# GATB/leon

Hardware: AMD Instinct MI355X
Metric: compressed input MB/s (DNA encode path) (higher is better)
Workload: dtype u64

## Files before the change

### leon_amd/csrc/host_rc.h

```cpp
#pragma once
#include <stdint.h>
#if defined(__x86_64__)
#include <emmintrin.h>
#define LEON_HOST_CHAIN_X86 1
#endif
#include <pthread.h>
#include <sched.h>
#if defined(__linux__)
#include <sys/mman.h>
#endif
#include <chrono>
#include <cstdio>
#include <condition_variable>
#include <cstdlib>
#include <cstring>
#include <new>
#include <algorithm>
#include <deque>
#include <memory>
#include <mutex>
#include <thread>
#include <type_traits>
#include <vector>

namespace leon {

class ReciprocalStream {
public:
    static constexpr uint64_t kChunk = 1ull << 18;
    static constexpr uint32_t kBufs = 12, kThreads = 3;
    ReciprocalStream() { for (auto& b : buf_) b.resize(kChunk); }
    ~ReciprocalStream() { stop(); }
    void restart() {
        stop();
        consumed_ = 0; quit_ = false;
        for (auto& h : holds_) h = 0;
        for (uint32_t j = 0; j < kThreads; j++) th_[j] = std::thread([this, j] { run(j); });
        running_ = true;
    }
    void stop() {
        if (!running_) return;
        { std::lock_guard<std::mutex> g(mu_); quit_ = true; }
        cv_.notify_all();
        for (auto& t : th_) t.join();
        running_ = false;
    }
    const uint64_t* take(uint64_t c) {
        std::unique_lock<std::mutex> g(mu_);
        if (c > consumed_) { consumed_ = c; cv_.notify_all(); }
        cv_.wait(g, [&] { return holds_[c % kBufs] == c + 1; });
        return buf_[c % kBufs].data();
    }
    static inline uint64_t reciprocal(uint64_t d) {
        if (d <= 256) return 0;
#ifdef LEON_HOST_CHAIN_X86
        uint64_t q, r;
        asm("divq %[d]" : "=a"(q), "=d"(r) : "a"(~0ull), "d"(255ull), [d] "r"(d) : "cc");
        return q;
#else
        return (uint64_t)(((((unsigned __int128)255) << 64) | ~0ull) / d);
#endif
    }
private:
    void run(uint32_t j) {
        for (uint64_t c = j;; c += kThreads) {
            {
                std::unique_lock<std::mutex> g(mu_);
                cv_.wait(g, [&] { return quit_ || c < consumed_ + kBufs; });
                if (quit_) return;
            }
            uint64_t* out = buf_[c % kBufs].data();
            const uint64_t t0 = c * kChunk;
            for (uint64_t i = 0; i < kChunk; i++) out[i] = reciprocal(5 + t0 + i);
            { std::lock_guard<std::mutex> g(mu_); holds_[c % kBufs] = c + 1; }
            cv_.notify_all();
        }
    }
    std::vector<uint64_t> buf_[kBufs];
    uint64_t holds_[kBufs] = {};
    std::mutex mu_;
    std::condition_variable cv_;
    uint64_t consumed_ = 0;
    bool quit_ = false, running_ = false;
    std::thread th_[kThreads];
};


struct ChainCpus {
    bool use = false;
    cpu_set_t set;
    void pick() {
        const char* e = getenv("LEON_CHAIN_PIN");
        if (!e || e[0] != '1') return;
        const int cpu = sched_getcpu();
        if (cpu < 0) return;
        char path[128];
        snprintf(path, sizeof path, "/sys/devices/system/cpu/cpu%d/cache/index3/shared_cpu_list", cpu);
        FILE* f = fopen(path, "r");
        if (!f) return;
        char line[1024];
        const bool ok = fgets(line, sizeof line, f) != nullptr;
        fclose(f);
        if (!ok) return;
        cpu_set_t l3, allowed;
        CPU_ZERO(&l3);
        for (char* p = line; *p && *p != '\n';) {
            char* q = nullptr;
            const long a = strtol(p, &q, 10);
            if (q == p) break;
            long b = a;
            if (*q == '-') { p = q + 1; b = strtol(p, &q, 10); }
            for (long c = a; c <= b && c < CPU_SETSIZE; c++) if (c >= 0) CPU_SET((int)c, &l3);
            p = *q == ',' ? q + 1 : q;
            if (*q != ',') break;
        }
        if (sched_getaffinity(0, sizeof allowed, &allowed) != 0) return;
        CPU_AND(&set, &l3, &allowed);
        use = CPU_COUNT(&set) >= 7;
    }
    void apply() const { if (use) (void)pthread_setaffinity_np(pthread_self(), sizeof set, &set); }
};

struct ChainRec16 { uint64_t c; uint32_t lo, fr; };
struct ChainRec24 { uint64_t c, lo, fr; };
struct ChainRecCarry { uint64_t c, qmm; uint32_t lo, fr; };

constexpr int kChainPrefetchBytes = 2048;

class ChainRing {
public:
    ChainRing() = default;
    ChainRing(const ChainRing&) = delete;
    ChainRing& operator=(const ChainRing&) = delete;
    ~ChainRing() { free(p_); }
    bool allocated() const { return p_ != nullptr; }
    size_t stride() const { return stride_; }
    void allocate(uint32_t n, size_t stride, bool huge) {
        constexpr size_t kHuge = (size_t)2 << 20;
        stride_ = (stride + 63) & ~(size_t)63;
        const size_t bytes = ((size_t)n * stride_ + kHuge - 1) & ~(kHuge - 1);
        void* q = nullptr;
        if (posix_memalign(&q, kHuge, bytes) != 0) throw std::bad_alloc();
        p_ = static_cast<char*>(q);
#if defined(__linux__) && defined(MADV_HUGEPAGE)
        if (huge) (void)madvise(p_, bytes, MADV_HUGEPAGE);
#else
        (void)huge;
#endif
    }
    void* at(uint32_t b) const { return p_ + (size_t)b * stride_; }
private:
    char* p_ = nullptr;
    size_t stride_ = 0;
};

class ChainFeed {
public:
    static constexpr uint32_t kMaxBufs = 1024;
    static constexpr uint64_t kPlainBelow = 512;
    struct View {
        const void* recs = nullptr; uint64_t n_syms = 0;
        bool wide = false, carry = false;
        const uint64_t* kmers = nullptr; uint32_t n_kmers = 0;
        uint64_t t0 = 0;
        uint64_t c_end[4] = {};
    };
    explicit ChainFeed(uint32_t k) : k_(k), W_(k >= 32 ? 2u : 1u), seg_kmers_(std::max<uint32_t>(1, (1u << 15) / k)) {
        carry_ = kCarryByDefault;
        if (const char* e = getenv("LEON_CHAIN_FORM")) { if (!strcmp(e, "carry")) carry_ = true; else if (!strcmp(e, "quotient")) carry_ = false; }
#ifdef LEON_HOST_CHAIN_X86
        if (carry_ && !__builtin_cpu_supports("bmi2")) carry_ = false;
#else
        carry_ = false;
#endif
        if (const char* e = getenv("LEON_CHAIN_HUGEPAGES")) huge_ = e[0] == '1';
        uint32_t n = carry_ ? 4 : 3, spares = 3;
        if (const char* e = getenv("LEON_CHAIN_HELPERS")) { const int v = atoi(e); if (v >= 1 && v <= 32) n = (uint32_t)v; }
        if (const char* e = getenv("LEON_CHAIN_SPARES")) { const int v = atoi(e); if (v >= 0 && v <= 32) spares = (uint32_t)v; }
        n_threads_ = n; n_spares_ = spares;
        if (const char* e = getenv("LEON_CHAIN_RING")) { const int v = atoi(e); if (v >= 4 && v <= (int)kMaxBufs) n_bufs_ = (uint32_t)v; }
    }
    ~ChainFeed() { stop(); }
    static constexpr bool kCarryByDefault = true;
    bool carry() const { return carry_; }
    ChainCpus cpus_;
    void start() {
        if (running_) return;
        quit_ = false;
        if (!ring_.allocated()) ring_.allocate(n_bufs_, (size_t)seg_kmers_ * k_ * (carry_ ? sizeof(ChainRecCarry) : sizeof(ChainRec16)), huge_);
        for (uint32_t j = 0; j < n_threads_ + n_spares_; j++) th_.emplace_back([this, j] { run(j >= n_threads_); });
        running_ = true;
    }
    void stop() {
        if (!running_) return;
        { std::lock_guard<std::mutex> g(mu_); quit_ = true; }
        cv_work_.notify_all(); cv_spare_.notify_all(); cv_ready_.notify_all();
        for (auto& t : th_) t.join();
        th_.clear();
        running_ = false;
    }
    void reset_stream() {
        std::lock_guard<std::mutex> g(mu_);
        segs_.clear(); base_ = 0; next_claim_ = 0; next_take_ = 0; released_ = 0; prefix_upto_ = 0; t_pushed_ = 0;
        for (auto& c : prefix_c_) c = 1;
        for (auto& r : ready_) r = 0;
    }
    uint32_t push(const uint64_t* kmers, size_t count) {
        uint32_t n = 0;
        {
            std::lock_guard<std::mutex> g(mu_);
            while (count) {
                const bool plain = t_pushed_ < kPlainBelow;
                const size_t take = plain ? std::min<size_t>(count, (kPlainBelow - t_pushed_ + k_ - 1) / k_) : std::min<size_t>(count, seg_kmers_);
                Seg sg; sg.kmers = kmers; sg.n_kmers = (uint32_t)take; sg.plain = plain; sg.t0 = t_pushed_;
                sg.wide = t_pushed_ + take * k_ + 8 >= (1ull << 32);
                segs_.push_back(sg);
                kmers += take * W_; count -= take; t_pushed_ += take * k_; n++;
            }
        }
        cv_work_.notify_all(); cv_spare_.notify_all();
        return n;
    }
    void take(View& v) {
        std::unique_lock<std::mutex> g(mu_);
        const uint64_t s = next_take_++;
        if (n_spares_ && (int64_t)(next_claim_ - next_take_) < (int64_t)low_water()) cv_spare_.notify_all();
        cv_ready_.wait(g, [&] { return ready_[s % n_bufs_] == s + 1; });
        const Seg& sg = segs_[s - base_];
        v.recs = sg.plain ? nullptr : slot(sg.wide, s);
        v.wide = sg.wide; v.carry = carry_ && !sg.wide;
        v.n_syms = (uint64_t)sg.n_kmers * k_; v.kmers = sg.kmers; v.n_kmers = sg.n_kmers; v.t0 = sg.t0;
        for (int i = 0; i < 4; i++) v.c_end[i] = sg.c_end[i];
    }
    void release() {
        { std::lock_guard<std::mutex> g(mu_); released_++; while (base_ < released_ && !segs_.empty()) { segs_.pop_front(); base_++; } }
        cv_work_.notify_all();
    }
private:
    struct Seg { const uint64_t* kmers; uint32_t n_kmers; bool plain, wide; uint64_t t0; uint64_t c0[4], c_end[4]; };
    static inline void count_codes(uint64_t x, uint64_t* n) {
        const uint64_t lo = x & 0x5555555555555555ull, hi = (x >> 1) & 0x5555555555555555ull;
        n[1] += (uint64_t)__builtin_popcountll(lo & ~hi); n[2] += (uint64_t)__builtin_popcountll(hi & ~lo); n[3] += (uint64_t)__builtin_popcountll(lo & hi);
    }
    uint64_t low_water() const { return n_bufs_ / 4; }
    void run(bool spare) {
        cpus_.apply();
        for (;;) {
            uint64_t s; Seg sg;
            {
                std::unique_lock<std::mutex> g(mu_);
                auto work = [&] { return next_claim_ < base_ + segs_.size() && next_claim_ < released_ + n_bufs_; };
                if (spare) cv_spare_.wait(g, [&] { return quit_ || (work() && (int64_t)(next_claim_ - next_take_) < (int64_t)low_water()); });
                else cv_work_.wait(g, [&] { return quit_ || work(); });
                if (quit_) return;
                s = next_claim_++;
                sg = segs_[s - base_];
            }
            uint64_t h[4] = {0, 0, 0, 0};
            for (uint32_t a = 0; a < sg.n_kmers; a++) for (uint32_t w = 0; w < W_; w++) count_codes(sg.kmers[(size_t)a * W_ + w], h);
            h[0] = (uint64_t)sg.n_kmers * k_ - h[1] - h[2] - h[3];
            uint64_t c[4];
            {
                std::unique_lock<std::mutex> g(mu_);
                cv_prefix_.wait(g, [&] { return quit_ || prefix_upto_ == s; });
                if (quit_) return;
                for (int i = 0; i < 4; i++) { c[i] = prefix_c_[i]; prefix_c_[i] += h[i]; }
                prefix_upto_ = s + 1;
                Seg& d = segs_[s - base_];
                for (int i = 0; i < 4; i++) { d.c0[i] = c[i]; d.c_end[i] = prefix_c_[i]; }
            }
            cv_prefix_.notify_all();
            if (!sg.plain) {
                if (sg.wide) {
                    { std::lock_guard<std::mutex> g(mu_); if (!wide_ring().allocated()) wide_ring_.allocate(n_bufs_, (size_t)seg_kmers_ * k_ * sizeof(ChainRec24), huge_); }
                    fill(static_cast<ChainRec24*>(slot(true, s)), sg, c);
                } else if (carry_) fill(static_cast<ChainRecCarry*>(slot(false, s)), sg, c);
                else fill(static_cast<ChainRec16*>(slot(false, s)), sg, c);
            }
            { std::lock_guard<std::mutex> g(mu_); ready_[s % n_bufs_] = s + 1; }
            cv_ready_.notify_all();
        }
    }
    static inline uint64_t scaled(uint64_t fr, uint64_t d) {
#ifdef LEON_HOST_CHAIN_X86
        uint64_t q, r;
        asm("divq %[d]" : "=a"(q), "=d"(r) : "a"(0ull), "d"(fr), [d] "r"(d) : "cc");
        return q;
#else
        return (uint64_t)((((unsigned __int128)fr) << 64) / d);
#endif
    }
    static inline uint64_t qmm_of(uint64_t fr) {
        constexpr uint64_t kNum = (1ull << 56) - 1;
        uint64_t m = (uint64_t)(int64_t)(0x1p56 / (double)(int64_t)fr);
        int64_t r = (int64_t)(kNum - m * fr);
        if (r < 0) { m--; r += (int64_t)fr; }
        if (r >= (int64_t)fr) { m++; r -= (int64_t)fr; }
        if (__builtin_expect((uint64_t)r >= fr, 0)) m = kNum / fr;
        return m;
    }
    template <typename Rec> void fill(Rec* out, const Seg& sg, uint64_t* c) const {
        uint64_t d = 5 + sg.t0 + 1;
        uint64_t cum[5] = {0, c[0], c[0] + c[1], c[0] + c[1] + c[2], c[0] + c[1] + c[2] + c[3]};
        for (uint32_t a = 0; a < sg.n_kmers; a++) {
            const uint64_t* w = sg.kmers + (size_t)a * W_;
            unsigned __int128 x = W_ == 2 ? (((unsigned __int128)w[1] << 64) | w[0]) << (128 - 2 * k_) : (unsigned __int128)w[0] << (128 - 2 * k_);
            for (uint32_t i = 0; i < k_; i++, d++, out++, x <<= 2) {
                const uint32_t sy = (uint32_t)(x >> 126);
                const uint64_t lo = cum[sy], fr = cum[sy + 1] - lo;
                out->c = scaled(fr, d);
                if constexpr (std::is_same<Rec, ChainRecCarry>::value) out->qmm = qmm_of(fr);
                out->lo = (decltype(out->lo))lo; out->fr = (decltype(out->fr))fr;
                cum[1] += sy < 1; cum[2] += sy < 2; cum[3] += sy < 3; cum[4]++;
            }
        }
        c[0] = cum[1]; c[1] = cum[2] - cum[1]; c[2] = cum[3] - cum[2]; c[3] = cum[4] - cum[3];
    }
    const uint32_t k_, W_, seg_kmers_;
    uint32_t n_threads_ = 5;
    ChainRing& wide_ring() { return ring_.stride() >= (size_t)seg_kmers_ * k_ * sizeof(ChainRec24) ? ring_ : wide_ring_; }
    void* slot(bool wide, uint64_t s) { return (wide ? wide_ring() : ring_).at((uint32_t)(s % n_bufs_)); }
    ChainRing ring_, wide_ring_;
    bool carry_ = false, huge_ = false;
    uint64_t ready_[kMaxBufs] = {};
    uint32_t n_bufs_ = 512, n_spares_ = 0;
    std::condition_variable cv_spare_;
    std::deque<Seg> segs_;
    uint64_t base_ = 0, next_claim_ = 0, next_take_ = 0, released_ = 0, prefix_upto_ = 0, t_pushed_ = 0;
    uint64_t prefix_c_[4] = {1, 1, 1, 1};
    std::mutex mu_;
    std::condition_variable cv_work_, cv_prefix_, cv_ready_;
    bool quit_ = false, running_ = false;
    std::vector<std::thread> th_;
};

class ByteBuf {
public:
    ~ByteBuf() { free(p_); }
    uint8_t* data() { return p_; }
    const uint8_t* data() const { return p_; }
    size_t size() const { return cap_; }
    void clear() {}
    void resize(size_t n) {
        if (n <= cap_) return;
        uint8_t* q = (uint8_t*)realloc(p_, n);
        if (!q) throw std::bad_alloc();
        p_ = q; cap_ = n;
    }
    uint8_t& operator[](size_t i) { return p_[i]; }
private:
    uint8_t* p_ = nullptr;
    size_t cap_ = 0;
};

class AnchorDictCoder {
public:
    AnchorDictCoder() { clear(); }
    void clear() {
        low_ = 0; range_ = ~0ull; n_ = 0; buf_.clear(); w_ = 0;
        for (int i = 0; i <= 5; i++) cum_[i] = i;
    }
    void encode_kmers(const uint64_t* w, size_t count, uint32_t k) {
        const uint32_t W = k >= 32 ? 2u : 1u;
        for (; count; count--, w += W) encode_kmer_plain(w, k);
    }
    inline void encode_kmer(const uint64_t* w, uint32_t k) { encode_kmers(w, 1, k); }
    inline void encode_kmer_plain(const uint64_t* w, uint32_t k) {
        if (buf_.size() < w_ + 8 * (size_t)k + 16) buf_.resize(buf_.size() * 2 + 8 * (size_t)k + 4096);
        for (uint32_t i = 0; i < k; i++) {
            const uint32_t bit = 2 * (k - 1 - i);
            encode((uint32_t)(w[bit >> 6] >> (bit & 63)) & 3u);
        }
    }
    void encode_segment(const ChainFeed::View& v, uint32_t k) {
#ifdef LEON_HOST_CHAIN_X86
        if (v.recs) {
            if (v.wide) encode_records(static_cast<const ChainRec24*>(v.recs), v.n_syms, v.t0);
            else if (v.carry) encode_records_carry(static_cast<const ChainRecCarry*>(v.recs), v.n_syms, v.t0);
            else encode_records(static_cast<const ChainRec16*>(v.recs), v.n_syms, v.t0);
            for (int i = 0; i < 4; i++) cum_[i + 1] = cum_[i] + v.c_end[i];
            cum_[5] = cum_[4] + 1;
            return;
        }
#endif
        encode_kmers(v.kmers, v.n_kmers, k);
    }
    void flush() {
        if (buf_.size() < w_ + 24) buf_.resize(w_ + 24);
        settle();
        for (int i = 0; i < 8; i++) { buf_[w_++] = (uint8_t)(low_ >> 56); low_ <<= 8; }
    }
    const uint8_t* data() const { return buf_.data(); }
    size_t size() const { return w_; }
    uint64_t symbols() const { return n_; }
private:
#ifdef LEON_HOST_CHAIN_X86
    template <typename Rec, int kAhead = kChainPrefetchBytes> void encode_records(const Rec* r, uint64_t n, uint64_t t0) {
        if (buf_.size() < w_ + 8 * n + 64) buf_.resize(buf_.size() * 2 + 8 * n + 4096);
        settle();
        uint8_t* p = buf_.data() + w_;
        uint8_t* p_end = buf_.data() + buf_.size() - 32;
        uint64_t L = low_, R = range_, tot1 = 5 + t0;
        uint64_t q = R / tot1;
        const Rec* const e = r + n;
        for (; r < e; r++) {
            tot1++;
            __builtin_prefetch(reinterpret_cast<const char*>(r) + kAhead);
            const uint64_t lo = r->lo, lf = lo + r->fr;
            const uint64_t Lu = L + q * lo;
            uint64_t Tu = L + q * lf;
            asm("" : "+r"(Tu));
            const uint64_t Ru = Tu - Lu, x = Lu ^ Tu;
            const uint64_t q8 = q << 8;
            const unsigned __int128 P = (unsigned __int128)q * r->c;
            const uint64_t Phi = (uint64_t)(P >> 64), Plo = (uint64_t)P, Phi8 = (Phi << 8) | (Plo >> 56), Plo8 = Plo << 8;
            if (__builtin_expect((x >> 48) == 0 || Ru < kBottom, 0)) {
                L = Lu; R = Ru;
                while ((L ^ (L + R)) < kTop || (R < kBottom && ((R = (0 - L) & (kBottom - 1)), true))) {
                    if (p >= p_end) { const size_t used = (size_t)(p - buf_.data()); buf_.resize(buf_.size() * 2 + 4096); p = buf_.data() + used; p_end = buf_.data() + buf_.size() - 32; }
                    *p++ = (uint8_t)(L >> 56);
                    R <<= 8;
                    L <<= 8;
                }
                q = R / tot1;
                continue;
            }
            uint64_t qn = Phi, Ln = Lu;
            R = Ru;
            *p = (uint8_t)(Lu >> 56);
            asm("cmpq %[top], %[x]\n\tcmovbq %[A], %[qn]\n\tcmovbq %[R1], %[R]\n\tcmovbq %[L1], %[Ln]\n\tadcq $0, %[p]"
                : [qn] "+r"(qn), [R] "+r"(R), [Ln] "+r"(Ln), [p] "+r"(p)
                : [x] "r"(x), [top] "r"(kTop), [A] "r"(Phi8), [R1] "r"(Ru << 8), [L1] "r"(Lu << 8)
                : "cc");
            if (__builtin_expect((Plo + q < q) | (Plo8 + q8 < q8), 0)) qn = R / tot1;
            q = qn; L = Ln;
        }
        w_ = (size_t)(p - buf_.data());
        low_ = L; range_ = R; n_ += n;
    }
    struct PlainStep { uint64_t q, L, R; uint8_t* p; };
    __attribute__((noinline)) PlainStep step_plain(const ChainRecCarry* r, uint64_t tot_next, uint64_t q, uint64_t L, uint8_t* p) {
        uint64_t Lo = L + q * r->lo, R = q * r->fr;
        uint8_t* p_end = buf_.data() + buf_.size() - 32;
        while ((Lo ^ (Lo + R)) < kTop || (R < kBottom && ((R = (0 - Lo) & (kBottom - 1)), true))) {
            if (p >= p_end) { const size_t used = (size_t)(p - buf_.data()); buf_.resize(buf_.size() * 2 + 4096); p = buf_.data() + used; p_end = buf_.data() + buf_.size() - 32; }
            *p++ = (uint8_t)(Lo >> 56);
            R <<= 8;
            Lo <<= 8;
        }
        return PlainStep{R / tot_next, Lo, R, p};
    }
#define LEON_CARRY_STEP(OFF, LIN, LOUT, LOUT32, EXIT)                                                                  \
                "movq  %%rdx, %%r14\n\t"                                  \
                "mulxq " OFF "(%[r]), %%rbx, %%rbx\n\t"                                                         \
                "movl  " OFF "+16(%[r]), " LOUT32 "\n\t"                                                         \
                "movl  " OFF "+20(%[r]), %%r13d\n\t"                                                             \
                "shlxq %[eight], " LOUT ", %%r12\n\t"                                                       \
                "shlxq %[eight], %%r13, %%r13\n\t"                                                          \
                "imulq %%rdx, %%r12\n\t"                                                              \
                "imulq %%rdx, %%r13\n\t"                                                         \
                "imulq %%rdx, " LOUT "\n\t"                                                                  \
                "cmpq  %%rdx, " OFF "+8(%[r])\n\t"                          \
                "sbbq  %%rax, %%rax\n\t"                                                                               \
                "orq   %%rax, %%r13\n\t"                                                              \
                "shlxq %[eight], %%rdx, %%rax\n\t"                                                               \
                "mulq  " OFF "(%[r])\n\t"                                            \
                "cmpq  %[dbt], %%rax\n\t"                                                                              \
                "ja    " EXIT "\n\t"                                                              \
                "shlxq %[eight], " LIN ", %%rax\n\t"                                                         \
                "addq  %%rax, %%r12\n\t"                                                    \
                "addq  " LIN ", " LOUT "\n\t"                                                                    \
                "cmpq  %[top], %%r13\n\t"                                                                              \
                "jb    " EXIT "\n\t"                                                               \
                "rorxq $56, " LOUT ", %%rax\n\t"                                                                       \
                "movb  %%al, (%[p])\n\t"                                     \
                "stc\n\t"                                                                                              \
                "adcq  %%r12, %%r13\n\t"                            \
                "cmovcq %%rbx, %%rdx\n\t"                                        \
                "cmovncq %%r12, " LOUT "\n\t"                                          \
                "sbbq  $-1, %[p]\n\t"
    template <int kAhead = kChainPrefetchBytes> void encode_records_carry(const ChainRecCarry* r, uint64_t n, uint64_t t0) {
        if (!n) return;
        if (buf_.size() < w_ + 8 * n + 64) buf_.resize(buf_.size() * 2 + 8 * n + 4096);
        settle();
        uint8_t* p = buf_.data() + w_;
        uint64_t L = low_;
        const ChainRecCarry* const r0 = r;
        uint64_t q = range_ / (5 + t0);
        const ChainRecCarry* const e = r + n - 1;
        const ChainRecCarry* const e2 = e - 1;
        const uint64_t doubt_above = ~(uint64_t)((((unsigned __int128)1) << 72) / (5 + t0));
        while (r < e) {
            if (r < e2) {
                asm volatile(
                    ".p2align 5\n"
                    "1:\n\t"
                    LEON_CARRY_STEP("0", "%[L]", "%%rcx", "%%ecx", "2f")
                    LEON_CARRY_STEP("24", "%%rcx", "%[L]", "%k[L]", "3f")
                    "prefetcht0 %c[ahead](%[r])\n\t"
                    "addq  $48, %[r]\n\t"
                    "cmpq  %[e], %[r]\n\t"
                    "jb    1b\n\t"
                    "jmp   4f\n"
                    "3:\n\t"
                    "movq  %%rcx, %[L]\n\t"
                    "addq  $24, %[r]\n"
                    "2:\n\t"
                    "movq  %%r14, %%rdx\n"
                    "4:\n"
                    : [r] "+r"(r), [q] "+d"(q), [L] "+r"(L), [p] "+r"(p)
                    : [e] "m"(e2), [top] "r"(kTop), [dbt] "r"(doubt_above), [eight] "r"((uint64_t)8), [ahead] "i"(kAhead)
                    : "rax", "rbx", "rcx", "r12", "r13", "r14", "cc", "memory");
            }
            if (r >= e) break;
            const PlainStep s = step_plain(r, 5 + t0 + (uint64_t)(r - r0) + 1, q, L, p);
            q = s.q; L = s.L; p = s.p;
            r++;
        }
        const PlainStep s = step_plain(r, 5 + t0 + n, q, L, p);
        w_ = (size_t)(s.p - buf_.data());
        low_ = s.L; range_ = s.R; n_ += n;
    }
#undef LEON_CARRY_STEP
#endif
    inline void settle() {
        uint8_t* p = buf_.data() + w_;
        while ((low_ ^ (low_ + range_)) < kTop || (range_ < kBottom && ((range_ = (0 - low_) & (kBottom - 1)), true))) {
            *p++ = (uint8_t)(low_ >> 56);
            range_ <<= 8;
            low_ <<= 8;
        }
        w_ = (size_t)(p - buf_.data());
    }
    inline void encode(uint32_t c) {
        settle();
        const uint64_t lo = cum_[c], fr = cum_[c + 1] - cum_[c], tot = cum_[5];
        const uint64_t q = range_ / tot;
        low_ += lo * q;
        range_ = q * fr;
        for (uint32_t i = 1; i <= 5; i++) cum_[i] += (uint64_t)(i > c);
        n_++;
    }
    static constexpr uint64_t kTop = 1ull << 56, kBottom = 1ull << 48;
    uint64_t low_, range_, n_, cum_[6];
    ByteBuf buf_;
    size_t w_;
};

inline bool decode_anchor_dict(const uint8_t* p, uint64_t n, uint64_t n_anchors, uint32_t k, uint64_t* out) {
    constexpr uint64_t kTop = 1ull << 56, kBottom = 1ull << 48;
    const uint32_t W = k >= 32 ? 2u : 1u;
    uint64_t low = 0, range = ~0ull, code = 0, i = 0, t = 0, cum[6] = {0, 1, 2, 3, 4, 5};
    for (int b = 0; b < 8; b++) code = (code << 8) | (i < n ? p[i] : 0), i++;
    ReciprocalStream recips;
    const bool use_inv = n_anchors * (uint64_t)k > (1u << 16);
    if (use_inv) recips.restart();
    const uint64_t* inv = nullptr;
    uint64_t inv_chunk = ~0ull;
    auto recip_of_symbol = [&](uint64_t tt) -> uint64_t {
        const uint64_t c = tt / ReciprocalStream::kChunk;
        if (c != inv_chunk) { inv = recips.take(c); inv_chunk = c; }
        return inv[tt % ReciprocalStream::kChunk];
    };
    auto next_byte = [&]() -> uint64_t { const uint64_t v = i < n ? p[i] : 0; i++; return v; };
    uint64_t r = 0;
    bool r_valid = false;
    for (uint64_t a = 0; a < n_anchors; a++) {
        unsigned __int128 km = 0;
        for (uint32_t j = 0; j < k; j++, t++) {
            const uint64_t tot = 5 + t;
            if (!r_valid) r = range / tot;
            if (r == 0) return false;
            const uint64_t d = code - low;
            const uint64_t p1 = r * cum[1], p2 = r * cum[2], p3 = r * cum[3], p4 = r * cum[4];
            const bool g1 = d >= p1, g2 = d >= p2, g3 = d >= p3, g4 = d >= p4;
            if (g4) return false;
            const uint64_t R0 = p1, R1 = p2 - p1, R2 = p3 - p2, R3 = p4 - p3;
            const uint32_t c = (uint32_t)g1 + (uint32_t)g2 + (uint32_t)g3;
            uint64_t lo, R, h = 0;
            const bool fast = use_inv && t >= 256;
            if (fast) {
                const uint64_t m1 = recip_of_symbol(t + 1);
                uint64_t h0 = (uint64_t)(((unsigned __int128)R0 * m1) >> 64), h1 = (uint64_t)(((unsigned __int128)R1 * m1) >> 64);
                uint64_t h2 = (uint64_t)(((unsigned __int128)R2 * m1) >> 64), h3 = (uint64_t)(((unsigned __int128)R3 * m1) >> 64);
                const uint64_t lo_a = g1 ? p1 : 0, R_a = g1 ? R1 : R0, h_a = g1 ? h1 : h0;
                const uint64_t lo_b = g3 ? p3 : p2, R_b = g3 ? R3 : R2, h_b = g3 ? h3 : h2;
                lo = g2 ? lo_b : lo_a; R = g2 ? R_b : R_a; h = g2 ? h_b : h_a;
            } else {
                lo = g3 ? p3 : g2 ? p2 : g1 ? p1 : 0;
                R = g3 ? R3 : g2 ? R2 : g1 ? R1 : R0;
            }
            low += lo;
            range = R;
            const uint64_t x = low ^ (low + range);
            if (__builtin_expect(!fast || (x >> 48) == 0 || range < kBottom, 0)) {
                while ((low ^ (low + range)) < kTop || (range < kBottom && ((range = (0 - low) & (kBottom - 1)), true))) {
                    code = (code << 8) | next_byte();
                    range <<= 8;
                    low <<= 8;
                    if (i > n + 16) return false;
                }
                r_valid = false;
            } else {
                const uint64_t byte = i < n ? p[i] : 0;
                const uint64_t tot1 = tot + 1;
                uint64_t rn = h >> 8;
#ifdef LEON_HOST_CHAIN_X86
                asm("cmpq %[top], %[x]\n\tcmovbq %[h], %[rn]\n\tcmovbq %[R8], %[rg]\n\tcmovbq %[L8], %[lw]\n\tcmovbq %[C8], %[cd]\n\tadcq $0, %[i]"
                    : [rn] "+r"(rn), [rg] "+r"(range), [lw] "+r"(low), [cd] "+r"(code), [i] "+r"(i)
                    : [x] "r"(x), [top] "r"(kTop), [h] "r"(h), [R8] "r"(range << 8), [L8] "r"(low << 8), [C8] "r"((code << 8) | byte)
                    : "cc");
#else
                const bool one = x < kTop;
                rn = one ? h : rn; range = one ? range << 8 : range; low = one ? low << 8 : low; code = one ? (code << 8) | byte : code; i += one;
#endif
                if (__builtin_expect(range - rn * tot1 >= tot1, 0)) rn++;
                r = rn; r_valid = true;
            }
            cum[1] += (uint64_t)(c < 1); cum[2] += (uint64_t)(c < 2); cum[3] += (uint64_t)(c < 3); cum[4] += 1; cum[5] += 1;
            km = (km << 2) | c;
        }
        out[a * W] = (uint64_t)km;
        if (W == 2) out[a * W + 1] = (uint64_t)(km >> 64);
    }
    return true;
}

class AnchorDictWorker {
public:
    explicit AnchorDictWorker(uint32_t k) : k_(k), feed_(k) {}
    ~AnchorDictWorker() { stop(); feed_.stop(); }
    void push(std::vector<uint64_t>&& kmers) {
        const uint32_t W = k_ >= 32 ? 2u : 1u;
        {
            std::lock_guard<std::mutex> g(mu_);
            if (!running_) { running_ = true; quit_ = false; feed_.cpus_.pick(); feed_.start(); th_ = std::thread([this] { feed_.cpus_.apply(); run(); }); }
            q_.emplace_back(std::move(kmers), 0u);
            q_.back().second = feed_.push(q_.back().first.data(), q_.back().first.size() / W);
            pending_++;
        }
        cv_.notify_all();
    }
    void drain() {
        std::unique_lock<std::mutex> g(mu_);
        cv_done_.wait(g, [this] { return pending_ == 0; });
    }
    void stop() {
        {
            std::lock_guard<std::mutex> g(mu_);
            if (!running_) return;
            quit_ = true;
        }
        cv_.notify_all();
        th_.join();
        running_ = false;
    }
    void reset() { drain(); coder_.clear(); feed_.reset_stream(); busy_ms_ = 0; starved_ms_ = 0; }
    double busy_ms() const { return busy_ms_; }
    double starved_ms() const { return starved_ms_; }
    AnchorDictCoder& coder() { return coder_; }
private:
    void run() {
        for (;;) {
            std::pair<std::vector<uint64_t>, uint32_t> batch;
            {
                std::unique_lock<std::mutex> g(mu_);
                cv_.wait(g, [this] { return quit_ || !q_.empty(); });
                if (q_.empty()) return;
                batch = std::move(q_.front());
                q_.pop_front();
            }
            const auto t0 = std::chrono::steady_clock::now();
            for (uint32_t sgm = 0; sgm < batch.second; sgm++) {
                ChainFeed::View v;
                const auto tw = std::chrono::steady_clock::now();
                feed_.take(v);
                starved_ms_ += std::chrono::duration<double, std::milli>(std::chrono::steady_clock::now() - tw).count();
                coder_.encode_segment(v, k_);
                feed_.release();
            }
            busy_ms_ += std::chrono::duration<double, std::milli>(std::chrono::steady_clock::now() - t0).count();
            {
                std::lock_guard<std::mutex> g(mu_);
                pending_--;
            }
            cv_done_.notify_all();
        }
    }
    uint32_t k_;
    ChainFeed feed_;
    AnchorDictCoder coder_;
    std::mutex mu_;
    std::condition_variable cv_, cv_done_;
    std::deque<std::pair<std::vector<uint64_t>, uint32_t>> q_;
    uint64_t pending_ = 0;
    double busy_ms_ = 0, starved_ms_ = 0;
    bool running_ = false, quit_ = false;
    std::thread th_;
};

}
```

Before: 20680.

## Add shifted-quotient chain record form with new asm encode loop as default

Adds a third precomputed record form in which the quotient-multiplier is stored pre-shifted by 8 bits with low bits set, plus a hand-written inline-asm range-coder step that carries the quotient left-shifted. This removes shift instructions from the serial encode dependency chain and folds the renormalisation into fewer ops. The new form becomes the default. The risk is subtle arithmetic correctness in the new asm, with slow-path fallbacks when the quotient estimate is in doubt.

```diff
diff --git a/leon_amd/csrc/host_rc.h b/leon_amd/csrc/host_rc.h
--- a/leon_amd/csrc/host_rc.h
+++ b/leon_amd/csrc/host_rc.h
@@ -124,6 +124,8 @@
 struct ChainRec16 { uint64_t c; uint32_t lo, fr; };
 struct ChainRec24 { uint64_t c, lo, fr; };
 struct ChainRecCarry { uint64_t c, qmm; uint32_t lo, fr; };
+struct ChainRecShifted { uint64_t c, qmm8; uint32_t lo, fr; };
+enum class ChainForm { quotient, carry, shifted };
 
 constexpr int kChainPrefetchBytes = 2048;
 
@@ -160,34 +162,36 @@
     static constexpr uint64_t kPlainBelow = 512;
     struct View {
         const void* recs = nullptr; uint64_t n_syms = 0;
-        bool wide = false, carry = false;
+        bool wide = false; ChainForm form = ChainForm::quotient;
         const uint64_t* kmers = nullptr; uint32_t n_kmers = 0;
         uint64_t t0 = 0;
         uint64_t c_end[4] = {};
     };
     explicit ChainFeed(uint32_t k) : k_(k), W_(k >= 32 ? 2u : 1u), seg_kmers_(std::max<uint32_t>(1, (1u << 15) / k)) {
-        carry_ = kCarryByDefault;
-        if (const char* e = getenv("LEON_CHAIN_FORM")) { if (!strcmp(e, "carry")) carry_ = true; else if (!strcmp(e, "quotient")) carry_ = false; }
+        form_ = kDefaultForm;
+        if (const char* e = getenv("LEON_CHAIN_FORM")) {
+            if (!strcmp(e, "shifted")) form_ = ChainForm::shifted; else if (!strcmp(e, "carry")) form_ = ChainForm::carry; else if (!strcmp(e, "quotient")) form_ = ChainForm::quotient;
+        }
 #ifdef LEON_HOST_CHAIN_X86
-        if (carry_ && !__builtin_cpu_supports("bmi2")) carry_ = false;
+        if (form_ != ChainForm::quotient && !__builtin_cpu_supports("bmi2")) form_ = ChainForm::quotient;
 #else
-        carry_ = false;
+        form_ = ChainForm::quotient;
 #endif
         if (const char* e = getenv("LEON_CHAIN_HUGEPAGES")) huge_ = e[0] == '1';
-        uint32_t n = carry_ ? 4 : 3, spares = 3;
+        uint32_t n = form_ != ChainForm::quotient ? 4 : 3, spares = 3;
         if (const char* e = getenv("LEON_CHAIN_HELPERS")) { const int v = atoi(e); if (v >= 1 && v <= 32) n = (uint32_t)v; }
         if (const char* e = getenv("LEON_CHAIN_SPARES")) { const int v = atoi(e); if (v >= 0 && v <= 32) spares = (uint32_t)v; }
         n_threads_ = n; n_spares_ = spares;
         if (const char* e = getenv("LEON_CHAIN_RING")) { const int v = atoi(e); if (v >= 4 && v <= (int)kMaxBufs) n_bufs_ = (uint32_t)v; }
     }
     ~ChainFeed() { stop(); }
-    static constexpr bool kCarryByDefault = true;
-    bool carry() const { return carry_; }
+    static constexpr ChainForm kDefaultForm = ChainForm::shifted;
+    ChainForm form() const { return form_; }
     ChainCpus cpus_;
     void start() {
         if (running_) return;
         quit_ = false;
-        if (!ring_.allocated()) ring_.allocate(n_bufs_, (size_t)seg_kmers_ * k_ * (carry_ ? sizeof(ChainRecCarry) : sizeof(ChainRec16)), huge_);
+        if (!ring_.allocated()) ring_.allocate(n_bufs_, (size_t)seg_kmers_ * k_ * (form_ != ChainForm::quotient ? sizeof(ChainRecCarry) : sizeof(ChainRec16)), huge_);
         for (uint32_t j = 0; j < n_threads_ + n_spares_; j++) th_.emplace_back([this, j] { run(j >= n_threads_); });
         running_ = true;
     }
@@ -228,7 +232,7 @@
         cv_ready_.wait(g, [&] { return ready_[s % n_bufs_] == s + 1; });
         const Seg& sg = segs_[s - base_];
         v.recs = sg.plain ? nullptr : slot(sg.wide, s);
-        v.wide = sg.wide; v.carry = carry_ && !sg.wide;
+        v.wide = sg.wide; v.form = form_;
         v.n_syms = (uint64_t)sg.n_kmers * k_; v.kmers = sg.kmers; v.n_kmers = sg.n_kmers; v.t0 = sg.t0;
         for (int i = 0; i < 4; i++) v.c_end[i] = sg.c_end[i];
     }
@@ -274,7 +278,8 @@
                 if (sg.wide) {
                     { std::lock_guard<std::mutex> g(mu_); if (!wide_ring().allocated()) wide_ring_.allocate(n_bufs_, (size_t)seg_kmers_ * k_ * sizeof(ChainRec24), huge_); }
                     fill(static_cast<ChainRec24*>(slot(true, s)), sg, c);
-                } else if (carry_) fill(static_cast<ChainRecCarry*>(slot(false, s)), sg, c);
+                } else if (form_ == ChainForm::shifted) fill(static_cast<ChainRecShifted*>(slot(false, s)), sg, c);
+                else if (form_ == ChainForm::carry) fill(static_cast<ChainRecCarry*>(slot(false, s)), sg, c);
                 else fill(static_cast<ChainRec16*>(slot(false, s)), sg, c);
             }
             { std::lock_guard<std::mutex> g(mu_); ready_[s % n_bufs_] = s + 1; }
@@ -310,6 +315,7 @@
                 const uint64_t lo = cum[sy], fr = cum[sy + 1] - lo;
                 out->c = scaled(fr, d);
                 if constexpr (std::is_same<Rec, ChainRecCarry>::value) out->qmm = qmm_of(fr);
+                if constexpr (std::is_same<Rec, ChainRecShifted>::value) out->qmm8 = (qmm_of(fr) << 8) | 255;
                 out->lo = (decltype(out->lo))lo; out->fr = (decltype(out->fr))fr;
                 cum[1] += sy < 1; cum[2] += sy < 2; cum[3] += sy < 3; cum[4]++;
             }
@@ -321,7 +327,8 @@
     ChainRing& wide_ring() { return ring_.stride() >= (size_t)seg_kmers_ * k_ * sizeof(ChainRec24) ? ring_ : wide_ring_; }
     void* slot(bool wide, uint64_t s) { return (wide ? wide_ring() : ring_).at((uint32_t)(s % n_bufs_)); }
     ChainRing ring_, wide_ring_;
-    bool carry_ = false, huge_ = false;
+    ChainForm form_ = ChainForm::quotient;
+    bool huge_ = false;
     uint64_t ready_[kMaxBufs] = {};
     uint32_t n_bufs_ = 512, n_spares_ = 0;
     std::condition_variable cv_spare_;
@@ -376,7 +383,8 @@
 #ifdef LEON_HOST_CHAIN_X86
         if (v.recs) {
             if (v.wide) encode_records(static_cast<const ChainRec24*>(v.recs), v.n_syms, v.t0);
-            else if (v.carry) encode_records_carry(static_cast<const ChainRecCarry*>(v.recs), v.n_syms, v.t0);
+            else if (v.form == ChainForm::shifted) encode_records_shifted(static_cast<const ChainRecShifted*>(v.recs), v.n_syms, v.t0);
+            else if (v.form == ChainForm::carry) encode_records_carry(static_cast<const ChainRecCarry*>(v.recs), v.n_syms, v.t0);
             else encode_records(static_cast<const ChainRec16*>(v.recs), v.n_syms, v.t0);
             for (int i = 0; i < 4; i++) cum_[i + 1] = cum_[i] + v.c_end[i];
             cum_[5] = cum_[4] + 1;
@@ -439,7 +447,7 @@
         low_ = L; range_ = R; n_ += n;
     }
     struct PlainStep { uint64_t q, L, R; uint8_t* p; };
-    __attribute__((noinline)) PlainStep step_plain(const ChainRecCarry* r, uint64_t tot_next, uint64_t q, uint64_t L, uint8_t* p) {
+    template <typename Rec> __attribute__((noinline)) PlainStep step_plain(const Rec* r, uint64_t tot_next, uint64_t q, uint64_t L, uint8_t* p) {
         uint64_t Lo = L + q * r->lo, R = q * r->fr;
         uint8_t* p_end = buf_.data() + buf_.size() - 32;
         while ((Lo ^ (Lo + R)) < kTop || (R < kBottom && ((R = (0 - Lo) & (kBottom - 1)), true))) {
@@ -522,6 +530,74 @@
         low_ = s.L; range_ = s.R; n_ += n;
     }
 #undef LEON_CARRY_STEP
+#define LEON_SHIFTED_STEP(OFF, LIN, LOUT, LOUT32, EXIT)                                                                \
+                "mulxq " OFF "(%[r]), %%rax, %%rbx\n\t"                              \
+                "cmpq  %[dbt], %%rax\n\t"                                                                              \
+                "ja    " EXIT "\n\t"                                                              \
+                "movl  " OFF "+16(%[r]), " LOUT32 "\n\t"                                                         \
+                "movl  " OFF "+20(%[r]), %%r13d\n\t"                                                             \
+                "mulxq " LOUT ", " LOUT ", %%r12\n\t"                                      \
+                "imulq %%rdx, %%r13\n\t"                                                         \
+                "cmpq  %%rdx, " OFF "+8(%[r])\n\t"                         \
+                "sbbq  %%rax, %%rax\n\t"                                                                               \
+                "orq   %%rax, %%r13\n\t"                                                              \
+                "cmpq  %[top], %%r13\n\t"                                                                              \
+                "jb    " EXIT "\n\t"                                                               \
+                "shlxq %[eight], " LIN ", %%rax\n\t"                                                         \
+                "addq  " LOUT ", %%rax\n\t"                                                 \
+                "orq   %%r12, " LOUT "\n\t"                        \
+                "rorxq $8, " LOUT ", " LOUT "\n\t"                                 \
+                "addq  " LIN ", " LOUT "\n\t"                                                                    \
+                "rorxq $56, " LOUT ", %%r12\n\t"                                                                       \
+                "movb  %%r12b, (%[p])\n\t"                                   \
+                "shlxq %[eight], %%rbx, %%rdx\n\t"              \
+                "andq  $-256, %%rbx\n\t"                                                \
+                "stc\n\t"                                                                                              \
+                "adcq  %%rax, %%r13\n\t"                            \
+                "cmovcq %%rbx, %%rdx\n\t"                                                                        \
+                "cmovncq %%rax, " LOUT "\n\t"                                          \
+                "sbbq  $-1, %[p]\n\t"
+    template <int kAhead = kChainPrefetchBytes> void encode_records_shifted(const ChainRecShifted* r, uint64_t n, uint64_t t0) {
+        if (!n) return;
+        if (buf_.size() < w_ + 8 * n + 64) buf_.resize(buf_.size() * 2 + 8 * n + 4096);
+        settle();
+        uint8_t* p = buf_.data() + w_;
+        uint64_t L = low_;
+        const ChainRecShifted* const r0 = r;
+        uint64_t S = (range_ / (5 + t0)) << 8;
+        const ChainRecShifted* const e = r + n - 1;
+        const ChainRecShifted* const e2 = e - 1;
+        const uint64_t doubt_above = ~(uint64_t)((((unsigned __int128)1) << 72) / (5 + t0));
+        while (r < e) {
+            if (r < e2) {
+                asm volatile(
+                    ".p2align 5\n"
+                    "1:\n\t"
+                    LEON_SHIFTED_STEP("0", "%[L]", "%%rcx", "%%ecx", "4f")
+                    LEON_SHIFTED_STEP("24", "%%rcx", "%[L]", "%k[L]", "3f")
+                    "prefetcht0 %c[ahead](%[r])\n\t"
+                    "addq  $48, %[r]\n\t"
+                    "cmpq  %[e], %[r]\n\t"
+                    "jb    1b\n\t"
+                    "jmp   4f\n"
+                    "3:\n\t"
+                    "movq  %%rcx, %[L]\n\t"
+                    "addq  $24, %[r]\n"
+                    "4:\n"
+                    : [r] "+r"(r), [S] "+d"(S), [L] "+r"(L), [p] "+r"(p)
+                    : [e] "m"(e2), [top] "r"(kTop), [dbt] "r"(doubt_above), [eight] "r"((uint64_t)8), [ahead] "i"(kAhead)
+                    : "rax", "rbx", "rcx", "r12", "r13", "cc", "memory");
+            }
+            if (r >= e) break;
+            const PlainStep s = step_plain(r, 5 + t0 + (uint64_t)(r - r0) + 1, S >> 8, L, p);
+            S = s.q << 8; L = s.L; p = s.p;
+            r++;
+        }
+        const PlainStep s = step_plain(r, 5 + t0 + n, S >> 8, L, p);
+        w_ = (size_t)(s.p - buf_.data());
+        low_ = s.L; range_ = s.R; n_ += n;
+    }
+#undef LEON_SHIFTED_STEP
 #endif
     inline void settle() {
         uint8_t* p = buf_.data() + w_;
```

Result: no change. 20710, median of 3 (+0.2%).
